# prime-slam/octreelib

Measured on AMD Instinct MI355X. Metric: Mpoints/s insert+subdivide+RANSAC, higher is better.
Workload: dtype f64; 1 GPU; BASELINE config 3: Grid 1 m voxels, 10000000 planar points per GPU (scene 32x32x32 voxels), insert + subdivide(len>64) + map_leaf_points_cuda_ransac(H=1024, k=6, thr=0.01, poses_per_batch=10) incl. apply_mask; points_per_gpu=10000000, K=64, hypotheses=1024, leaves=575543

## Files before the change

### octreelib_amd/csrc/common.h

```cpp
#pragma once

#include <hip/hip_runtime.h>
#include <stdint.h>

#include <cstdio>
#include <cstring>
#include <map>
#include <string>
#include <vector>

#include "../../include/octreelib_hip.h"

#include <atomic>
extern std::atomic<uint64_t> g_octl_host_syncs;
static inline hipError_t octl_counted_stream_sync(hipStream_t s) {
  g_octl_host_syncs.fetch_add(1, std::memory_order_relaxed);
  return hipStreamSynchronize(s);
}
static inline hipError_t octl_counted_event_sync(hipEvent_t e) {
  g_octl_host_syncs.fetch_add(1, std::memory_order_relaxed);
  return hipEventSynchronize(e);
}
#define hipStreamSynchronize(s) octl_counted_stream_sync(s)
#define hipEventSynchronize(e) octl_counted_event_sync(e)
// ... 51 lines not shown
  int64_t no_fused_tables = 0;
  int64_t no_spin_wait = 0;
  int64_t ransac_waves = 0;
  int64_t geom_margin = 0;
  int64_t no_ransac_prescreen = 0;
  int64_t no_spec_finish = 0;
};
int64_t* octl_option_field(OctlOptions& o, const char* name);

struct octl_ctx {
  int device = 0;
  OctlOptions opt;
  hipStream_t stream = nullptr;
  std::string err;
  int profiling = 0;
  std::map<std::string, KernelTiming> timings;
  std::vector<PendingEvent> pending;
  std::vector<hipEvent_t> event_pool;
  DevBuf scan_tmp[3];
  DevBuf scan_status;
  uint32_t scan_epoch = 0;
  int cus = 0;
  DevBuf small;
  void* small_host = nullptr;
  void* pinned = nullptr;
  hipEvent_t pin_event[3] = {nullptr, nullptr, nullptr};
  hipEvent_t handoff_event = nullptr;
  hipStream_t copy_stream = nullptr;
  hipEvent_t copy_gate = nullptr;
  hipStream_t self_stream = nullptr;
  hipEvent_t self_gate = nullptr, self_done = nullptr;
  struct Upload { const char* dst; size_t bytes; hipEvent_t done; };
  std::vector<Upload> uploads;
  std::vector<DevBuf> pool;
  size_t pool_bytes = 0;
  std::map<void*, size_t> user_blocks;
  unsigned char geom_hint[192] = {0};
  bool geom_hint_valid = false;
  bool geom_hint_staged = false;
  struct octl_forest* pending_mask_forest = nullptr;
  uint64_t geom_hint_want = 0;
  bool geom_hint_two_pass = false;
  bool geom_sparse = false;
  bool had_chunks = false;
  int64_t spec_points = 0, spec_nodes = 0, spec_vox = 0, spec_blocks = 0;
  DevBuf hyp_dev;
  DevBuf f32_stage;
  DevBuf ls_buf;
  DevBuf rs_counters;
  int rs_parity = 0;
  uint32_t wait_seq = 0;
  bool rs_counters_dirty = false;
  std::vector<double> hyp_host;
  void* comm = nullptr;
  int n_ranks = 1, rank = 0;
  DevBuf routed_xyz, routed_gidx;
  bool routed_taken = false;
  DevBuf rt_hist, rt_counts, rt_matrix, rt_send_xyz, rt_send_gidx;
  int64_t routed_n = 0;
};

int octl_set_error(octl_ctx* ctx, int code, const char* fmt, ...);
enum { MIRROR_COPY_WORDS = 512, MIRROR_BBOX_WORD = 896, MIRROR_RS_VIOLATION = 990, MIRROR_MASK_TOTALS = 992,
       MIRROR_FLAG_BUILD = 1000, MIRROR_FLAG_MASK0 = 1001, MIRROR_FLAG_MASK1 = 1002 };
static_assert(MIRROR_COPY_WORDS <= MIRROR_BBOX_WORD && MIRROR_BBOX_WORD + 8 <= MIRROR_RS_VIOLATION &&
              MIRROR_RS_VIOLATION < MIRROR_MASK_TOTALS &&
              MIRROR_MASK_TOTALS + 2 <= MIRROR_FLAG_BUILD && MIRROR_FLAG_MASK1 < 1024, "mirror layout");
enum {
  SM_ERR = 0,
  SM_BBOX = 4,
  SM_NVOX = 12,
  SM_NSPLIT = 13,
  SM_NTILES = 14,
  SM_ETOTAL = 15,
  SM_NBLOCKS = 16,
  SM_BK_TICKET = 17,
  SM_BK_OVERFULL = 18,
  SM_SLOT_VOXELS = 21,
  SM_MASK_TOTAL = 22,
  SM_BK_NOORDER = 23,
  SM_DEBUG_TOTAL = 24,
  SM_BK_FLAGS = 25,
  SM_BK_TOTAL = 26,
  SM_BK_TODO = 27,
  SM_BK_MISSING = 28,
  SM_CK_COUNT = 29,
  SM_INC_MISS = 28,
  SM_INC_BAD = 29,
  SM_INC_DEAD = 30,
  SM_INC_NEWVOX = 31,
  SM_SLOT_COUNTS = 28,
  SM_BUILD_WORDS = 32,
  SM_BK_LEVEL = 40,
  SM_GEOM = 64,
  SM_SLOT_HIST = 64,
  SM_ALLREDUCE = 512,
  SM_WORDS = 1024
};
static_assert(SM_ERR < SM_BUILD_WORDS && SM_BBOX + 6 <= SM_BUILD_WORDS && SM_NVOX < SM_BUILD_WORDS &&
                  SM_NSPLIT < SM_BUILD_WORDS && SM_NTILES < SM_BUILD_WORDS && SM_ETOTAL < SM_BUILD_WORDS &&
                  SM_NBLOCKS < SM_BUILD_WORDS && SM_BK_TICKET < SM_BUILD_WORDS && SM_BK_OVERFULL < SM_BUILD_WORDS &&
                  SM_SLOT_VOXELS < SM_BUILD_WORDS && SM_MASK_TOTAL < SM_BUILD_WORDS &&
                  SM_BK_NOORDER < SM_BUILD_WORDS && SM_DEBUG_TOTAL < SM_BUILD_WORDS && SM_BK_FLAGS < SM_BUILD_WORDS &&
                  SM_BK_TOTAL < SM_BUILD_WORDS && SM_BK_TODO < SM_BUILD_WORDS && SM_BK_MISSING < SM_BUILD_WORDS &&
                  SM_CK_COUNT < SM_BUILD_WORDS && SM_INC_NEWVOX < SM_BUILD_WORDS &&
                  SM_SLOT_COUNTS + 4 <= SM_BUILD_WORDS,
// ... 90 lines not shown
```

### octreelib_amd/csrc/ctx.hip

```cpp
#include <chrono>
#include <cstdarg>
#include <cstdlib>

#include <algorithm>

#include "common.h"

int octl_set_error(octl_ctx* ctx, int code, const char* fmt, ...) {
  char buf[1024];
  va_list ap;
  va_start(ap, fmt);
  vsnprintf(buf, sizeof(buf), fmt, ap);
  va_end(ap);
  if (ctx) ctx->err = buf;
  return code;
}

std::atomic<uint64_t> g_octl_host_syncs{0};

namespace {
struct OptName { const char* name; int64_t OctlOptions::*field; };
const OptName kOptions[] = {
    {"NO_BUCKET_BUILD", &OctlOptions::no_bucket_build},     {"BUCKET_POINTS", &OctlOptions::bucket_points},
    {"SYNC_GEOM", &OctlOptions::sync_geom},                 {"NO_GEOM_HINT", &OctlOptions::no_geom_hint},
// ... 315 lines not shown
  if (!out) return OCTL_E_INVALID;
  *out = nullptr;
  int n = 0;
  if (hipGetDeviceCount(&n) != hipSuccess || n <= 0 || device_id < 0 || device_id >= n)
    return OCTL_E_HIP;
  if (hipSetDevice(device_id) != hipSuccess) return OCTL_E_HIP;
  octl_ctx* ctx = new octl_ctx();
  ctx->device = device_id;
  options_from_environment(ctx->opt);
  if (hipStreamCreateWithFlags(&ctx->stream, hipStreamNonBlocking) != hipSuccess) {
    delete ctx;
    return OCTL_E_HIP;
  }
  if (hipMalloc(&ctx->small.p, 4096) != hipSuccess ||
      hipHostMalloc(&ctx->small_host, 4096, hipHostMallocDefault) != hipSuccess ||
      hipHostMalloc(&ctx->pinned, OCTL_PINNED_BYTES, hipHostMallocDefault) != hipSuccess) {
    if (ctx->small.p) (void)hipFree(ctx->small.p);
    (void)hipStreamDestroy(ctx->stream);
    delete ctx;
    return OCTL_E_NOMEM;
  }
  ctx->small.cap = 4096;
  std::memset(ctx->small_host, 0, 4096);
  (void)hipMemsetAsync(ctx->small.p, 0, 4096, ctx->stream);
  (void)hipStreamSynchronize(ctx->stream);
  *out = ctx;
  return OCTL_OK;
}

int octl_comm_destroy(octl_ctx* ctx);

void octl_ctx_destroy(octl_ctx* ctx) {
  if (!ctx) return;
  (void)hipSetDevice(ctx->device);
  (void)hipStreamSynchronize(ctx->stream);
  if (ctx->comm) (void)octl_comm_destroy(ctx);
  for (auto& pe : ctx->pending) {
    (void)hipEventDestroy(pe.start);
    (void)hipEventDestroy(pe.stop);
  }
  for (auto ev : ctx->event_pool) (void)hipEventDestroy(ev);
  if (ctx->handoff_event) (void)hipEventDestroy(ctx->handoff_event);
  for (auto ev : ctx->pin_event)
    if (ev) (void)hipEventDestroy(ev);
  for (auto& pb : ctx->pool) (void)hipFree(pb.p);
  ctx->pool.clear();
  for (auto& ub : ctx->user_blocks) (void)hipFree(ub.first);
  ctx->user_blocks.clear();
  for (auto& b : ctx->scan_tmp) devbuf_free(b);
  devbuf_free(ctx->hyp_dev);
  devbuf_free(ctx->f32_stage);
  devbuf_free(ctx->ls_buf);
  devbuf_free(ctx->rs_counters);
  devbuf_free(ctx->scan_status);
  devbuf_free(ctx->small);
  devbuf_free(ctx->routed_xyz);
  devbuf_free(ctx->routed_gidx);
  for (DevBuf* b : {&ctx->rt_hist, &ctx->rt_counts, &ctx->rt_matrix, &ctx->rt_send_xyz,
                    &ctx->rt_send_gidx})
    devbuf_free(*b);
  if (ctx->small_host) (void)hipHostFree(ctx->small_host);
  if (ctx->pinned) (void)hipHostFree(ctx->pinned);
  if (ctx->self_stream) {
    (void)hipStreamSynchronize(ctx->self_stream);
    (void)hipStreamDestroy(ctx->self_stream);
    if (ctx->self_gate) (void)hipEventDestroy(ctx->self_gate);
    if (ctx->self_done) (void)hipEventDestroy(ctx->self_done);
  }
  if (ctx->copy_stream) {
    (void)hipStreamSynchronize(ctx->copy_stream);
    (void)hipStreamDestroy(ctx->copy_stream);
  }
  if (ctx->copy_gate) (void)hipEventDestroy(ctx->copy_gate);
  for (auto& u : ctx->uploads) (void)hipEventDestroy(u.done);
  (void)hipStreamDestroy(ctx->stream);
  delete ctx;
}

const char* octl_last_error(const octl_ctx* ctx) { return ctx ? ctx->err.c_str() : "null context"; }

int octl_ctx_sync(octl_ctx* ctx) {
  if (!ctx) return OCTL_E_INVALID;
  HIP_TRY(ctx, hipStreamSynchronize(ctx->stream));
  return mirror_check_violation(ctx);
}

int octl_host_alloc(octl_ctx* ctx, int64_t bytes, void** p) {
  if (!ctx || !p || bytes < 0) return OCTL_E_INVALID;
  (void)hipSetDevice(ctx->device);
  hipError_t e = hipHostMalloc(p, (size_t)(bytes > 0 ? bytes : 1), hipHostMallocDefault);
  if (e != hipSuccess)
    return octl_set_error(ctx, OCTL_E_NOMEM, "hipHostMalloc(%lld) failed: %s", (long long)bytes, hipGetErrorString(e));
  return OCTL_OK;
}

int octl_host_free(octl_ctx* ctx, void* p) {
  if (!ctx) return OCTL_E_INVALID;
  if (ctx->copy_stream) (void)hipStreamSynchronize(ctx->copy_stream);
  if (p) HIP_TRY(ctx, hipHostFree(p));
  return OCTL_OK;
}

int octl_dev_upload_async(octl_ctx* ctx, void* dptr, const void* src, int64_t bytes) {
  if (!ctx || bytes < 0 || (bytes > 0 && (!dptr || !src))) return OCTL_E_INVALID;
  HIP_TRY(ctx, hipSetDevice(ctx->device));
  if (!ctx->copy_stream) {
// ... 130 lines not shown
```

### octreelib_amd/csrc/order.hip

```cpp
#include <algorithm>

#include "forest.h"

namespace {

__global__ __launch_bounds__(256) void k_sub_up(const int32_t* __restrict__ first_child,
                                                int64_t a, int64_t b,
                                                uint32_t* __restrict__ nint) {
  const int64_t x = a + (int64_t)blockIdx.x * blockDim.x + threadIdx.x;
  if (x >= b) return;
  const int32_t fc = first_child[x];
  uint32_t s = 0;
  if (fc >= 0) {
    s = 1;
#pragma unroll
    for (int j = 0; j < 8; ++j) s += nint[fc + j];
  }
  nint[x] = s;
}

__global__ __launch_bounds__(256) void k_rank_down(const int32_t* __restrict__ first_child,
                                                   int64_t a, int64_t b,
                                                   const uint32_t* __restrict__ nint,
                                                   uint32_t* __restrict__ rank) {
// ... 263 lines not shown
  OCTL_TRY(forest_settle(f));
  octl_ctx* ctx = f->ctx;
  if (!f->built) return octl_set_error(ctx, OCTL_E_STATE, "no scheme has been built");
  const int n_poses = (int)f->pose_off.size() - 1;
  if (e0 && n_e0 != n_poses) return octl_set_error(ctx, OCTL_E_INVALID, "e0 size mismatch");
  std::vector<uint32_t> slot_counts;
  OCTL_TRY(forest_reference_order(f, e0, slot_counts, false));
  *n_blocks = f->n_blocks;
  const int64_t n = std::min<int64_t>(cap, f->n_blocks);
  if (n > 0 && order) {
    HIP_TRY(ctx, hipMemcpyAsync(order, f->rs_order.p, (size_t)n * 4, hipMemcpyDeviceToHost,
                                ctx->stream));
    HIP_TRY(ctx, hipStreamSynchronize(ctx->stream));
  }
  return OCTL_OK;
}

static int ransac_all_impl(octl_forest* f, int32_t poses_per_batch, const int32_t* e0, int32_t n_e0,
                           const double* hypotheses, int32_t H, int32_t k, double threshold,
                           bool* mask_fresh);

extern "C" int octl_forest_ransac_all(octl_forest* f, int32_t poses_per_batch, const int32_t* e0,
                                      int32_t n_e0, const double* hypotheses, int32_t H, int32_t k,
                                      double threshold) {
  if (!f || !hypotheses) return OCTL_E_INVALID;
  OCTL_TRY(forest_settle(f));
  bool mask_fresh = false;
  const int rc = ransac_all_impl(f, poses_per_batch, e0, n_e0, hypotheses, H, k, threshold, &mask_fresh);
  if (mask_fresh) f->mask_valid = (rc == OCTL_OK);
  return rc;
}

static int ransac_all_impl(octl_forest* f, int32_t poses_per_batch, const int32_t* e0, int32_t n_e0,
                           const double* hypotheses, int32_t H, int32_t k, double threshold,
                           bool* mask_fresh) {
  octl_ctx* ctx = f->ctx;
  if (!f->built) return octl_set_error(ctx, OCTL_E_STATE, "ransac before build");
  if (poses_per_batch < 1) return octl_set_error(ctx, OCTL_E_INVALID, "poses_per_batch < 1");
  if (H < 1 || H > 1024 || k < 1) return octl_set_error(ctx, OCTL_E_INVALID, "bad H or k");
  OCTL_TRY(ransac_check_table(ctx, hypotheses, H, k));
  const int n_poses = (int)f->pose_off.size() - 1;
  if (e0 && n_e0 != n_poses) return octl_set_error(ctx, OCTL_E_INVALID, "e0 size mismatch");
  HIP_TRY(ctx, hipSetDevice(ctx->device));
  hipStream_t st = ctx->stream;
  if (!f->mask_valid) {
    OCTL_TRY(devbuf_reserve(ctx, f->mask, (size_t)std::max<int64_t>(f->n_ord, 1)));
    *mask_fresh = true;
  }
  if (f->n_blocks == 0) return OCTL_OK;
  const size_t hyp_cap_before = ctx->hyp_dev.cap;
  OCTL_TRY(devbuf_reserve(ctx, ctx->hyp_dev, (size_t)H * k * 8));
  const bool same_table = hyp_cap_before == ctx->hyp_dev.cap && ctx->hyp_host.size() == (size_t)H * k &&
                          std::memcmp(ctx->hyp_host.data(), hypotheses, (size_t)H * k * 8) == 0;
  if (same_table) {
  } else if ((size_t)H * k * 8 <= 64 * 1024) {
    char* pin = static_cast<char*>(ctx->pinned) + 128 * 1024;
    OCTL_TRY(pin_region_wait(ctx, 1));
    std::memcpy(pin, hypotheses, (size_t)H * k * 8);
    OCTL_TRY(octl_copy_from_pinned(ctx, ctx->hyp_dev.p, pin, (size_t)H * k * 8));
    OCTL_TRY(pin_region_mark(ctx, 1));
  } else {
    HIP_TRY(ctx, hipMemcpyAsync(ctx->hyp_dev.p, hypotheses, (size_t)H * k * 8, hipMemcpyHostToDevice, st));
    HIP_TRY(ctx, hipStreamSynchronize(st));
  }
  if (!same_table) ctx->hyp_host.assign(hypotheses, hypotheses + (size_t)H * k);
  const bool one_batch = n_poses <= poses_per_batch;
  std::vector<uint32_t> slot_counts;
  OCTL_TRY(forest_reference_order(f, e0, slot_counts, !one_batch));
  if (one_batch) {
    OCTL_TRY(ransac_launch(ctx, f->xyz_ord.as<double>(), f->n_ord, f->blk_start.as<uint32_t>(),
                           f->blk_size.as<int32_t>(), f->rs_order.as<int32_t>(), f->n_blocks,
                           ctx->hyp_dev.as<double>(), H, k, threshold, f->mask.as<uint8_t>(), nullptr,
                           nullptr, nullptr, nullptr, f->rs_scratch, f->max_block_hint));
    return OCTL_OK;
  }
  int64_t off = 0;
  for (int p0 = 0; p0 < n_poses; p0 += poses_per_batch) {
    int64_t nbatch = 0;
    for (int p = p0; p < std::min(n_poses, p0 + poses_per_batch); ++p) nbatch += slot_counts[p];
    if (nbatch > 0)
      OCTL_TRY(ransac_launch(ctx, f->xyz_ord.as<double>(), f->n_ord, f->blk_start.as<uint32_t>(),
                             f->blk_size.as<int32_t>(), f->rs_order.as<int32_t>() + off, nbatch,
                             ctx->hyp_dev.as<double>(), H, k, threshold, f->mask.as<uint8_t>(),
                             nullptr, nullptr, nullptr, nullptr, f->rs_scratch, f->max_block_hint));
    off += nbatch;
  }
  return OCTL_OK;
}
```

### octreelib_amd/csrc/ransac.hip

```cpp
#include <algorithm>
#include <cstdlib>
#include <type_traits>

#include "forest.h"
#include "lookback.h"
#include "plane_cert.h"
#include "wave_utils.h"

namespace {

__device__ __forceinline__ double div_by_small_int(double c, int k) {
  const double kd = (double)k;
  const double zh = 1.0 / kd;
  const double zl = fma(-kd, zh, 1.0) / kd;
  const double a = fabs(c);
  if (!((int(a > 1e-290) | int(c == 0.0)) & int(a < 1e290))) return c / kd;
  return copysign(fma(c, zh, c * zl), c);
}

__device__ __forceinline__ bool coord_in_fast_range(double v) {
  const uint32_t hi = (uint32_t)__double2hiint(v), lo = (uint32_t)__double2loint(v);
  const uint32_t e = (hi >> 20) & 0x7FFu;
  return (e - (1023u - 30u)) <= 60u || (hi | lo) == 0u;
}
// ... 276 lines not shown
  }
  unsigned long long best = 0;
#pragma unroll
  for (int q = 0; q < HPL; ++q) {
    const int t = threadIdx.x + q * THREADS;
    if (t < H) {
      const unsigned long long key =
          ((unsigned long long)(unsigned)cnt[q] << 32) | (unsigned)(0x7FFFFFFF - t);
      best = key > best ? key : best;
    }
  }
#pragma unroll
  for (int off = 32; off > 0; off >>= 1) {
    const unsigned long long o = __shfl_xor(best, off);
    best = o > best ? o : best;
  }
  if ((threadIdx.x & 63) == 0) s_best[threadIdx.x >> 6] = best;
  __syncthreads();
  best = s_best[0];
#pragma unroll
  for (int w = 1; w < THREADS / 64; ++w) best = s_best[w] > best ? s_best[w] : best;
  const int win = 0x7FFFFFFF - (int)(unsigned)(best & 0xFFFFFFFFu);
#pragma unroll
  for (int q = 0; q < HPL; ++q) {
    if ((int)threadIdx.x + q * THREADS == win) {
      const float f0 = (float)pa[q], f1 = (float)pb[q], f2 = (float)pc[q], f3 = (float)pd[q];
      s_plane[0] = f0; s_plane[1] = f1; s_plane[2] = f2; s_plane[3] = f3;
      if (out.plane) {
        out.plane[4 * (int64_t)be + 0] = f0; out.plane[4 * (int64_t)be + 1] = f1;
        out.plane[4 * (int64_t)be + 2] = f2; out.plane[4 * (int64_t)be + 3] = f3;
      }
      if (out.count) out.count[be] = cnt[q];
      if (out.index) out.index[be] = win;
    }
  }
  __syncthreads();
  const double a = (double)s_plane[0], bb = (double)s_plane[1], c = (double)s_plane[2],
               dd = (double)s_plane[3];
  for (int i = threadIdx.x; i < n; i += THREADS)
    out.mask[pstart + i] = (plane_distance(a, bb, c, dd, pts[3 * (int64_t)i], pts[3 * (int64_t)i + 1],
                                           pts[3 * (int64_t)i + 2]) < thr) ? 1 : 0;
}

typedef float f4 __attribute__((ext_vector_type(4)));
__device__ __forceinline__ float fma32(float a, float b, float c) { return __builtin_fmaf(a, b, c); }
__device__ __forceinline__ float min3abs(float m, float a, float b) {
  float r;
  asm("v_min3_f32 %0, %1, |%2|, |%3|" : "=v"(r) : "v"(m), "v"(a), "v"(b));
  return r;
}

template <int CTRL, int ROW_MASK>
__device__ __forceinline__ uint32_t dpp_u32(uint32_t v) {
  return (uint32_t)__builtin_amdgcn_update_dpp((int)v, (int)v, CTRL, ROW_MASK, 0xF, false);
}
__device__ __forceinline__ uint32_t wave_max_u32(uint32_t v) {
  v = max(v, dpp_u32<0xB1, 0xF>(v));
  v = max(v, dpp_u32<0x4E, 0xF>(v));
  v = max(v, dpp_u32<0x141, 0xF>(v));
  v = max(v, dpp_u32<0x140, 0xF>(v));
  v = max(v, dpp_u32<0x142, 0xA>(v));
  v = max(v, dpp_u32<0x143, 0xC>(v));
  return (uint32_t)__builtin_amdgcn_readlane((int)v, 63);
}
__device__ __forceinline__ float wave_max_nonneg_f32(float m) {
  return __uint_as_float(wave_max_u32(__float_as_uint(m)));
}

template <int CTRL, int ROW_MASK>
__device__ __forceinline__ double dpp_f64_or_zero(double v) {
  const int lo = __builtin_amdgcn_update_dpp(0, __double2loint(v), CTRL, ROW_MASK, 0xF, false);
  const int hi = __builtin_amdgcn_update_dpp(0, __double2hiint(v), CTRL, ROW_MASK, 0xF, false);
  return __hiloint2double(hi, lo);
}
__device__ __forceinline__ double wave_sum_f64(double v) {
  v += dpp_f64_or_zero<0xB1, 0xF>(v);
  v += dpp_f64_or_zero<0x4E, 0xF>(v);
  v += dpp_f64_or_zero<0x141, 0xF>(v);
  v += dpp_f64_or_zero<0x140, 0xF>(v);
  v += dpp_f64_or_zero<0x142, 0xA>(v);
  v += dpp_f64_or_zero<0x143, 0xC>(v);
  return __hiloint2double(__builtin_amdgcn_readlane(__double2hiint(v), 63),
                          __builtin_amdgcn_readlane(__double2loint(v), 63));
}

template <int THREADS, bool SFAST = false>
__device__ __forceinline__ void stage_local(unsigned tx, double ox, double oy, double oz, const BlockDesc& d,
                                            double px, double py, double pz, f4* loc,
                                            float* wext, uint32_t* wfast, float* ext_out = nullptr,
                                            uint32_t* fast_out = nullptr) {
  float m = 0.f;
  if ((int)tx < d.n) {
    const float u = (float)(px - ox), v = (float)(py - oy), w = (float)(pz - oz);
    loc[tx] = f4{u, v, w, 0.f};
    m = fmaxf(fabsf(u), fmaxf(fabsf(v), fabsf(w)));
    if (!(m == m) || u != u || v != v || w != w) m = __int_as_float(0x7f800000);
  }
  m = wave_max_nonneg_f32(m);
  const bool inr = coord_in_fast_range(px) && coord_in_fast_range(py) && coord_in_fast_range(pz);
  const bool wave_fast = __all(inr);
  if (ext_out) {
    *ext_out = m;
    *fast_out = SFAST ? (uint32_t)__builtin_amdgcn_readfirstlane(wave_fast ? 1 : 0) : (wave_fast ? 1u : 0u);
  } else if ((tx & 63) == 0) {
    wext[tx >> 6] = m;
    wfast[tx >> 6] = wave_fast ? 1u : 0u;
  }
}

template <int NH>
__device__ __forceinline__ void screen_group(const f4* __restrict__ loc, int n, const float* fa,
                                             const float* fb, const float* fc, const float* sto,
                                             float nthr2, int* cnt, float* margin) {
  float mg[2][NH];
#pragma unroll
  for (int h = 0; h < NH; ++h) mg[0][h] = mg[1][h] = __int_as_float(0x7f800000);
  for (int base = 0; base < n; base += 32) {
    const int m = __builtin_amdgcn_readfirstlane(min(32, n - base));
    uint32_t hist[NH];
#pragma unroll
    for (int h = 0; h < NH; ++h) hist[h] = 0;
    auto score = [&](const f4 L, float (&e)[NH]) {
#pragma unroll
      for (int h = 0; h < NH; ++h) {
        const float sv = fma32(fa[h], L.x, fma32(fb[h], L.y, fma32(fc[h], L.z, sto[h])));
        e[h] = fma32(sv, sv, nthr2);
        hist[h] = __builtin_amdgcn_alignbit(hist[h], __float_as_uint(e[h]), 31);
      }
    };
    int i = 0;
    for (; i + 4 <= m; i += 4) {
      const f4 L0 = loc[base + i], L1 = loc[base + i + 1], L2 = loc[base + i + 2],
               L3 = loc[base + i + 3];
      float e0[NH], e1[NH], e2[NH], e3[NH];
// ... 454 lines not shown
              RS_COUNT(17, 64 * (n - m1));
              RS_COUNT(21, 1);
              survive(mine && c2[0] > Lcur, (uint32_t)c2[0], (int)(w & 1023u));
              qhead += nq;
            };
            auto prescreen = [&](auto nh_tag, const int qb) {
              constexpr int NH = decltype(nh_tag)::value;
              uint2 pe[NH];
              auto hyp_a = [&](const int h) { return (int)tx + (qb + h) * THREADS; };
#pragma unroll
              for (int h = 0; h < NH; ++h)
                pe[h] = pos_tab[(size_t)n * (size_t)H + (size_t)((FULLH || hyp_a(h) < H) ? hyp_a(h) : 0)];
              float qa[NH], qb_[NH], qc[NH], qto[NH], qT2[NH];
              bool qok[NH];
              int qcnt[NH];
              uint32_t risk = 0;
#pragma unroll
              for (int h = 0; h < NH; ++h) {
                const uint32_t w0 = pe[h].x, w1 = pe[h].y;
                f4 P[KS];
#pragma unroll
                for (int i = 0; i < KS; ++i) P[i] = loc[((i < 4 ? w0 : w1) >> (8 * (i & 3))) & 0xFFu];
                const float inv_k = 1.0f / (float)KS;
                float cx = P[0].x, cy = P[0].y, cz = P[0].z;
#pragma unroll
                for (int i = 1; i < KS; ++i) {
                  cx += P[i].x;
                  cy += P[i].y;
                  cz += P[i].z;
                }
                cx *= inv_k;
                cy *= inv_k;
                cz *= inv_k;
                float xx, xy, xz, yy, yz, zz;
                {
                  const float ax = P[0].x - cx, ay = P[0].y - cy, az = P[0].z - cz;
                  xx = ax * ax; xy = ax * ay; xz = ax * az; yy = ay * ay; yz = ay * az; zz = az * az;
                }
#pragma unroll
                for (int i = 1; i < KS; ++i) {
                  const float ax = P[i].x - cx, ay = P[i].y - cy, az = P[i].z - cz;
                  xx = fma32(ax, ax, xx); xy = fma32(ax, ay, xy); xz = fma32(ax, az, xz);
                  yy = fma32(ay, ay, yy); yz = fma32(ay, az, yz); zz = fma32(az, az, zz);
                }
                const float dx = fma32(yy, zz, -(yz * yz)), dy = fma32(xx, zz, -(xz * xz)), dz = fma32(xx, yy, -(xy * xy));
                const float cA = fma32(xz, yz, -(xy * zz)), cB = fma32(xy, yz, -(xz * yy)), cC = fma32(xy, xz, -(yz * xx));
                const bool is_x = dx > dy && dx > dz;
                const bool is_y = !is_x && dy > dz;
                const float m1 = is_x ? dx : (is_y ? cA : cB);
                const float m2 = is_x ? cA : (is_y ? dy : cC);
                const float m3 = is_x ? cB : (is_y ? cC : dz);
                const float ss = fma32(m3, m3, fma32(m2, m2, m1 * m1));
                const float r = __builtin_amdgcn_rsqf(ss);
                const float a = m1 * r, b = m2 * r, c = m3 * r;
                qa[h] = a; qb_[h] = b; qc[h] = c;
                float to = -fma32(c, cz, fma32(b, cy, a * cx));
                asm volatile("" : "+v"(to));
                qto[h] = to;
                const float T = (xx + yy) + zz;
                const float mu4 = fma32(fma32(pc.qa, T, pc.qb), T, pc.qc);
                const float gap = __builtin_fmaxf(__builtin_fmaxf(dx, dy), dz) - __builtin_amdgcn_fmed3f(dx, dy, dz);
                qok[h] = (ss * r > mu4) && (gap > mu4);
                risk |= w1;
                const float thr_h = fma32(pc.e35, mu4 * r, pc.thrblk);
                qT2[h] = thr_h * thr_h;
                qcnt[h] = 0;
              }
              if (__any((risk >> 16) != 0u)) {
#pragma unroll
                for (int h = 0; h < NH; ++h) qok[h] = qok[h] && (pe[h].y >> 16) == 0u;
              }
              RS_COUNT(12, NH);
              RS_COUNT(22, 64 * NH * n);
              if constexpr (TWO) {
                if (two_stage) {
                  bool bad = false;
#pragma unroll
                  for (int h = 0; h < NH; ++h) bad = bad || !qok[h];
                  if (__any(bad)) {
#pragma unroll
                    for (int h = 0; h < NH; ++h) {
                      if (!qok[h]) {
                        qa[h] = qb_[h] = qc[h] = qto[h] = 0.f;
                        qT2[h] = 1.f;
                      }
                    }
                  }
                  screen_ub<NH>(ploc, m1, qa, qb_, qc, qto, qT2, qcnt);
                  RS_COUNT(16, 64 * NH * m1);
#pragma unroll
                  for (int h = 0; h < NH; ++h) {
                    const bool alive = qcnt[h] > m1 - budget && (FULLH || hyp_a(h) < H);
                    const unsigned long long mk = __ballot(alive);
                    if (alive) {
                      const int e = (qtail + (int)__builtin_amdgcn_mbcnt_hi((uint32_t)(mk >> 32), __builtin_amdgcn_mbcnt_lo((uint32_t)mk, 0u))) &
                                    (RS_STAGE2_RING - 1);
                      qlo[e] = __float_as_uint(qa[h]);
                      qlo[RS_STAGE2_RING + e] = __float_as_uint(qb_[h]);
                      qlo[2 * RS_STAGE2_RING + e] = __float_as_uint(qc[h]);
                      qhi[e] = __float_as_uint(qto[h]);
                      qhi[RS_STAGE2_RING + e] = __float_as_uint(qT2[h]);
                      qhi[2 * RS_STAGE2_RING + e] = ((uint32_t)qcnt[h] << 10) | (uint32_t)hyp_a(h);
                    }
                    qtail += __popcll(mk);
                    RS_COUNT(18, __popcll(mk));
                    if (qtail - qhead >= 64) stage2(64);
                  }
                  return;
                }
              }
              screen_ub<NH>(loc, n, qa, qb_, qc, qto, qT2, qcnt);
              RS_COUNT(20, 64 * NH * n);
#pragma unroll
              for (int h = 0; h < NH; ++h)
                survive(!(qok[h] && qcnt[h] <= Lcur) && (FULLH || hyp_a(h) < H),
                        (THREADS == 64 && qok[h]) ? (uint32_t)qcnt[h] : 63u, hyp_a(h));
            };
            constexpr int PNH = 3;
            constexpr int TRIOS = (HPL - 1) / PNH, REST = (HPL - 1) % PNH;
            if (TWO && certified) {
              const float E = extent;
              const float G = ((float)(fabs(lx[0]) + fabs(ly[0]) + fabs(lz[0])) + E) * 0x1.0002p0f;
              const float E2 = E * E;
              const float floor2 = fma32(0x1p-74f * (G * G), E2, 0x1p-24f * (E2 * E2)) * 0x1.0002p0f;
              const uint32_t* __restrict__ trio = reinterpret_cast<const uint32_t*>(pos_tab) + trio_word(n, H, 0);
              auto trio_of = [&](int g) {
                const int t = (int)tx + g * THREADS;
                return trio[(FULLH || t < H) ? t : 0];
              };
              auto at = [&](uint32_t off) { return *reinterpret_cast<const f4*>(reinterpret_cast<const char*>(loc) + off); };
              uint32_t e_next = trio_of(1);
#pragma unroll 1
              for (int g = 1; g < HPL; ++g) {
                const int t = (int)tx + g * THREADS;
                const bool real = FULLH || t < H;
                const uint32_t e = e_next;
                e_next = trio_of(g + 1 < HPL ? g + 1 : g);
                const f4 P0 = at(e & 0x3F0u), P1 = at((e >> 10) & 0x3F0u), P2 = at((e >> 20) & 0x3F0u);
                const float ux = P1.x - P0.x, uy = P1.y - P0.y, uz = P1.z - P0.z;
                const float vx = P2.x - P0.x, vy = P2.y - P0.y, vz = P2.z - P0.z;
// ... 415 lines not shown
      sp = start[phys[r + 1]];
    } else if (!order) {
      const int64_t e = (int64_t)d.pstart + d.n;
      if (e < n_points) sp = (uint32_t)e;
    }
    d.pspill = sp;
    d.pad[0] = 0;
    d.pad[1] = (uint32_t)b;
    d.pad[2] = 0;
    desc[b] = d;
    if (d.n < k) {
      for (int i = 0; i < d.n; ++i) out.mask[(int64_t)d.pstart + i] = 0;
      if (out.plane) {
        out.plane[4 * b + 0] = 0.f; out.plane[4 * b + 1] = 0.f;
        out.plane[4 * b + 2] = 0.f; out.plane[4 * b + 3] = 0.f;
      }
      if (out.count) out.count[b] = 0;
      if (out.index) out.index[b] = -1;
    } else if (d.n > cap) {
      big_list[atomicAdd(&counters[RC_BIG], 1u)] = (uint32_t)b;
    } else {
      atomicAdd(&bins[d.n], 1u);
    }
    if (d.n >= k && (int64_t)d.n > max_block)
      __hip_atomic_store(&mirror[MIRROR_RS_VIOLATION], 1u, __ATOMIC_RELAXED, __HIP_MEMORY_SCOPE_SYSTEM);
  }
  __syncthreads();
  if (bins[threadIdx.x]) atomicAdd(&counters[RC_BINS + threadIdx.x], bins[threadIdx.x]);
}

__device__ __forceinline__ void pos_table_entry(const double* __restrict__ hyp, int H, int k,
                                                uint2* __restrict__ tab, int n, int t) {
  const double* __restrict__ row = hyp + (int64_t)t * k;
  uint32_t x = 0, y = 0;
  for (int i = 0; i < k; ++i) {
    bool risky;
    const uint32_t g = (uint32_t)sample_index_cached(row[i], n, &risky);
    if (i < 4) x |= g << (8 * i); else y |= g << (8 * (i - 4));
    y |= (risky || g == (uint32_t)n) ? (0x10000u << i) : 0u;
  }
  tab[(size_t)n * (size_t)H + t] = uint2{x, y};
  if (n < RS_TINY_THREADS && k >= 3) {
    auto p = [&](int i) { return ((i < 4 ? x : y) >> (8 * (i & 3))) & 0xFFu; };
    const uint32_t p0 = p(0);
    uint32_t p1 = p(k - 1), p2 = p(k - 1);
    for (int i = k - 2; i >= 1; --i) p1 = p(i) != p0 ? p(i) : p1;
    for (int i = k - 2; i >= 2; --i) p2 = (p(i) != p0 && p(i) != p1) ? p(i) : p2;
    const bool flagged = (y >> 16) != 0u || p1 == p0 || p2 == p0 || p2 == p1;
    reinterpret_cast<uint32_t*>(tab)[trio_word(n, H, t)] = flagged ? TRIO_FLAG : (p0 << 4) | (p1 << 14) | (p2 << 24);
  }
}
__device__ __forceinline__ void pos_table_part(const double* __restrict__ hyp, int H, int k,
                                               const uint32_t* __restrict__ counters, uint2* __restrict__ tab,
                                               int n, int part) {
  const int t = part * 256 + (int)threadIdx.x;
  if (t >= H || n < k || counters[RC_BINS + n] == 0u) return;
  pos_table_entry(hyp, H, k, tab, n, t);
}

__global__ __launch_bounds__(256) void k_block_scatter(const BlockDesc* __restrict__ desc, int64_t nb,
                                                       int cap, int k,
                                                       uint32_t* __restrict__ counters,
                                                       BlockDesc* __restrict__ sdesc, unsigned n_scatter,
                                                       const double* __restrict__ hyp, int H,
                                                       uint2* __restrict__ tab, uint32_t* __restrict__ next_counters) {
  if (next_counters && blockIdx.x == gridDim.x - 1)
    for (int w = threadIdx.x; w < RC_WORDS; w += blockDim.x) next_counters[w] = 0;
  if (blockIdx.x >= n_scatter) {
    const unsigned parts = (unsigned)(H + 255) / 256u;
    const unsigned id = blockIdx.x - n_scatter;
    pos_table_part(hyp, H, k, counters, tab, (int)(id / parts), (int)(id % parts));
    return;
  }
  __shared__ uint32_t cnt[256];
  __shared__ uint32_t base[256];
  __shared__ uint32_t c[256];
  cnt[threadIdx.x] = 0;
  c[threadIdx.x] = counters[RC_BINS + threadIdx.x];
  __syncthreads();
  uint32_t first = 0;
  for (int m = 255; m > (int)threadIdx.x; --m) first += c[m];
  if (blockIdx.x == 0) {
    counters[RC_START + threadIdx.x] = first;
    if (threadIdx.x == 0) counters[RC_SORTED] = first + c[0];
  }
  constexpr int PER_THREAD = BS_PER_THREAD;
  const int64_t b0 = (int64_t)blockIdx.x * (256 * PER_THREAD);
  int nn[PER_THREAD];
  uint32_t rank[PER_THREAD];
#pragma unroll
  for (int r = 0; r < PER_THREAD; ++r) {
    const int64_t b = b0 + r * 256 + threadIdx.x;
    nn[r] = -1;
    rank[r] = 0;
    if (b < nb) {
      const int n = desc[b].n;
      if (n >= k && n <= cap) {
        nn[r] = n;
        rank[r] = atomicAdd(&cnt[n], 1u);
      }
    }
  }
  __syncthreads();
  if (cnt[threadIdx.x]) base[threadIdx.x] = first + atomicAdd(&counters[RC_FILL + threadIdx.x], cnt[threadIdx.x]);
  __syncthreads();
#pragma unroll
  for (int r = 0; r < PER_THREAD; ++r) {
    if (nn[r] >= 0) {
      const int64_t b = b0 + r * 256 + threadIdx.x;
      sdesc[base[nn[r]] + rank[r]] = desc[b];
    }
  }
}

constexpr int BPS_THREADS = 1024, BPS_MAX = BPS_THREADS * 8;
template <int BPS_PER_THREAD>
__global__ __launch_bounds__(BPS_THREADS) void k_block_prepare_small(
    const int32_t* __restrict__ order, const uint32_t* __restrict__ start, const int32_t* __restrict__ size,
    int64_t nb, int64_t n_points, int cap, int k, BlockDesc* __restrict__ desc, BlockDesc* __restrict__ sdesc,
    uint32_t* __restrict__ big_list, uint32_t* __restrict__ counters, RansacOut out, int64_t max_block,
    uint32_t* __restrict__ mirror, const double* __restrict__ hyp, int H, uint2* __restrict__ tab,
    uint32_t* __restrict__ next_counters) {
  if (blockIdx.x > 0) {
    const int parts = (H + BPS_THREADS - 1) / BPS_THREADS;
// ... 86 lines not shown
  uint32_t cm = 0, incm = 0;
  if (threadIdx.x < 256) {
    cm = bins[255 - threadIdx.x];
    incm = wave_inclusive_add(cm);
    if (lane == 63) s_wave[wave] = incm;
  }
  __syncthreads();
  if (threadIdx.x < 256) {
    uint32_t f = incm - cm;
    for (int w = 0; w < wave; ++w) f += s_wave[w];
    const int m = 255 - (int)threadIdx.x;
    first[m] = f;
    counters[RC_BINS + m] = cm;
    counters[RC_START + m] = f;
    if (m == 0) counters[RC_SORTED] = f + cm;
  }
  __syncthreads();
#pragma unroll
  for (int r = 0; r < BPS_PER_THREAD; ++r)
    if (dd[r].n >= 0) sdesc[first[dd[r].n] + rank[r]] = dd[r];
}

}

int ransac_check_table(octl_ctx* ctx, const double* hyp, int32_t H, int32_t k) {
  const int64_t n = (int64_t)H * k;
  for (int64_t i = 0; i < n; ++i)
    if (!(hyp[i] >= 0.0 && hyp[i] < 1.0))
      return octl_set_error(ctx, OCTL_E_INVALID,
                            "hypothesis table entry %lld = %g is outside [0, 1): the table must hold "
                            "np.random.random draws (cuda_ransac.py:39-41)", (long long)i, hyp[i]);
  return OCTL_OK;
}

int ransac_launch(octl_ctx* ctx, const double* xyz_dev, int64_t n_points,
                  const uint32_t* blk_start, const int32_t* blk_size, const int32_t* order_dev,
                  int64_t nb, const double* hyp_dev, int32_t H, int32_t k, double thr,
                  uint8_t* mask_dev, float* plane_dev, int32_t* count_dev, int32_t* index_dev,
                  uint8_t* evaluated_dev, DevBuf& scratch, int64_t max_block) {
  (void)evaluated_dev;
  if (nb <= 0) return OCTL_OK;
  if (H < 1 || H > 1024) return octl_set_error(ctx, OCTL_E_INVALID, "H must be in [1, 1024]");
  if (k < 1) return octl_set_error(ctx, OCTL_E_INVALID, "initial_points_number must be positive");
  const bool any_k = k > RS_KMAX;
  if (nb >= ((int64_t)1 << 31)) return octl_set_error(ctx, OCTL_E_INVALID, "too many blocks");
  hipStream_t st = ctx->stream;
  const size_t off_d = (((size_t)nb + 8) * 4 + 31) & ~(size_t)31;
  const size_t off_s = off_d + (size_t)nb * sizeof(BlockDesc);
  const size_t off_b = off_s + (size_t)nb * sizeof(BlockDesc);
  const size_t off_c = (off_b + (size_t)nb * 4 + 31) & ~(size_t)31;
  const bool use_tab = !any_k && k >= 3 && k <= 6 && (H > 256 || k == 6);
  const size_t off_t = (off_c + RC_WORDS * 4 + 31) & ~(size_t)31;
  const size_t tab_bytes = (size_t)256 * (size_t)H * sizeof(uint2) + (size_t)RS_TINY_THREADS * (size_t)H * sizeof(uint32_t);
  OCTL_TRY(devbuf_reserve(ctx, scratch, off_t + (use_tab ? tab_bytes : 0)));
  char* base = static_cast<char*>(scratch.p);
  uint32_t* tmp = scratch.as<uint32_t>();
  BlockDesc* desc = reinterpret_cast<BlockDesc*>(base + off_d);
  BlockDesc* sdesc = reinterpret_cast<BlockDesc*>(base + off_s);
  uint32_t* big_list = reinterpret_cast<uint32_t*>(base + off_b);
  uint32_t* counters = reinterpret_cast<uint32_t*>(base + off_c);
  const bool fused = !ctx->opt.no_fused_tables;
  uint32_t* next_counters = nullptr;
  if (fused) {
    if (!ctx->rs_counters.p || ctx->rs_counters_dirty) {
      OCTL_TRY(devbuf_reserve(ctx, ctx->rs_counters, (size_t)2 * RC_WORDS * 4));
      HIP_TRY(ctx, hipMemsetAsync(ctx->rs_counters.p, 0, (size_t)2 * RC_WORDS * 4, st));
      ctx->rs_parity = 0;
    }
    counters = ctx->rs_counters.as<uint32_t>() + (size_t)ctx->rs_parity * RC_WORDS;
    next_counters = ctx->rs_counters.as<uint32_t>() + (size_t)(ctx->rs_parity ^ 1) * RC_WORDS;
    ctx->rs_parity ^= 1;
    ctx->rs_counters_dirty = true;
  }
  uint2* pos_tab = use_tab ? reinterpret_cast<uint2*>(base + off_t) : nullptr;
  const int threads = (H <= 64) ? 64 : (H <= 256 ? 256 : RS_BIG_THREADS);
  RansacOut out{mask_dev, plane_dev, count_dev, index_dev};
  if (fused && nb <= BPS_MAX) {
    KTimer t(ctx, "ransac_prepare");
    const int cap = any_k ? 0 : threads - 1;
    const unsigned n_table = use_tab && cap >= k ? (unsigned)(cap - k + 1) * (unsigned)ceil_div(H, BPS_THREADS) : 0u;
    auto kp = nb <= 2 * BPS_THREADS ? k_block_prepare_small<2>
              : (nb <= 4 * BPS_THREADS ? k_block_prepare_small<4>
                                       : (nb <= 6 * BPS_THREADS ? k_block_prepare_small<6> : k_block_prepare_small<8>));
    OCTL_LAUNCH(kp, dim3(1 + n_table), dim3(BPS_THREADS), 0, st, order_dev, blk_start, blk_size, nb,
                       n_points, cap, (int)k, desc, sdesc, big_list, counters, out, max_block,
                       static_cast<uint32_t*>(ctx->small_host), hyp_dev, (int)H, pos_tab, next_counters);
    HIP_TRY(ctx, hipGetLastError());
    ctx->rs_counters_dirty = false;
  } else {
    KTimer t(ctx, "ransac_prepare");
    if (fused) {
      const unsigned g = (unsigned)ceil_div(nb, 256 * BP_PER_THREAD);
      uint64_t* status = nullptr;
      uint32_t epoch = 0;
      OCTL_TRY(octl_scan_status_acquire(ctx, g, &status, &epoch));
      OCTL_LAUNCH(k_block_prepare, dim3(g), dim3(256), 0, st, order_dev, blk_start, blk_size, nb, n_points,
                         any_k ? 0 : threads - 1, (int)k, desc, big_list, counters, out, status, epoch, max_block,
                         static_cast<uint32_t*>(ctx->small_host));
      HIP_TRY(ctx, hipGetLastError());
    } else {
      const unsigned g = (unsigned)ceil_div(nb, 256);
      OCTL_LAUNCH(k_block_sizes_in_order, dim3(g), dim3(256), 0, st, order_dev, blk_size, nb, tmp, counters);
      HIP_TRY(ctx, hipGetLastError());
      OCTL_TRY(octl_exclusive_scan_u32(ctx, tmp, tmp, nb, nullptr));
      OCTL_LAUNCH(k_block_desc, dim3((unsigned)ceil_div(nb, 256 * BD_PER_THREAD)), dim3(256), 0, st, order_dev,
                         blk_start, blk_size,
                         (const uint32_t*)tmp, nb, n_points, any_k ? 0 : threads - 1, (int)k, desc, big_list,
                         counters, out);
      HIP_TRY(ctx, hipGetLastError());
    }
    const unsigned n_scatter = (unsigned)ceil_div(nb, 256 * BS_PER_THREAD);
    const unsigned n_table = use_tab ? 256u * (unsigned)ceil_div(H, 256) : 0u;
    OCTL_LAUNCH(k_block_scatter, dim3(n_scatter + n_table), dim3(256), 0, st,
                       (const BlockDesc*)desc, nb, any_k ? 0 : threads - 1, (int)k, counters, sdesc, n_scatter, hyp_dev,
                       (int)H, pos_tab, next_counters);
    HIP_TRY(ctx, hipGetLastError());
    ctx->rs_counters_dirty = false;
  }
  const int cus = octl_ctx_cus(ctx);
  KTimer t(ctx, "ransac");
  hipStream_t side = st;
  bool on_side = false;
  int waves_per_block = (int)ctx->opt.ransac_waves;
  if (waves_per_block == 0 && !any_k && H > 256) {
    const int64_t slots = (int64_t)cus * 16;
    if (nb * 2 <= slots) waves_per_block = 4;
    else if (nb <= 6 * slots) waves_per_block = 2;
  }
  const bool need_small = max_block >= RS_TINY_THREADS, need_mid = max_block >= RS_SMALL_THREADS,
             need_big = any_k || max_block >= threads;
  const bool side_work = waves_per_block == 4 ? need_big
                         : (waves_per_block == 2 ? (need_mid || need_big) : (need_small || need_mid || need_big));
  if (!any_k && H > 256 && side_work && octl_ctx_side_stream(ctx) &&
      hipEventRecord(ctx->self_gate, st) == hipSuccess &&
      hipStreamWaitEvent(ctx->self_stream, ctx->self_gate, 0) == hipSuccess) {
    side = ctx->self_stream;
    on_side = true;
  }
  const int no_prescreen = ctx->opt.no_ransac_prescreen ? 1 : 0;
#define OCTL_RANSAC_RANGE(THREADS, HPL, KT, PER_CU, LO, HI, PT, ST)                              \
  do {                                                                                           \
    const unsigned g = (unsigned)std::min<int64_t>(nb, (int64_t)cus * (PER_CU));                 \
    if (H == (THREADS) * (HPL))                                                                  \
      OCTL_LAUNCH((k_ransac<THREADS, HPL, KT, true, PT>), dim3(g), dim3(THREADS), 0, ST,         \
                         xyz_dev, (const BlockDesc*)sdesc, (const uint32_t*)(LO), (const uint32_t*)(HI), \
                         hyp_dev, H, k, thr, out, (const uint2*)pos_tab, no_prescreen);           \
    else                                                                                         \
      OCTL_LAUNCH((k_ransac<THREADS, HPL, KT, false, PT>), dim3(g), dim3(THREADS), 0, ST,        \
                         xyz_dev, (const BlockDesc*)sdesc, (const uint32_t*)(LO), (const uint32_t*)(HI), \
                         hyp_dev, H, k, thr, out, (const uint2*)pos_tab, no_prescreen);           \
  } while (0)
#define OCTL_RANSAC_LAUNCH(THREADS, HPL, KT, PER_CU, PT) \
  OCTL_RANSAC_RANGE(THREADS, HPL, KT, PER_CU, nullptr, counters + RC_SORTED, PT, st)
#define OCTL_RANSAC_SPLIT(KT)                                                                                    \
  do {                                                                                                           \
    if (waves_per_block == 4) {                                                                                  \
      OCTL_RANSAC_RANGE(RS_BIG_THREADS, RS_BIG_HPL, KT, RS_PER_CU, nullptr, counters + RC_SORTED, true, st);     \
    } else if (waves_per_block == 2) {                                                                           \
      if (need_mid)                                                                                              \
        OCTL_RANSAC_RANGE(RS_BIG_THREADS, RS_BIG_HPL, KT, RS_PER_CU, nullptr,                                    \
                          counters + RC_START + RS_SMALL_THREADS - 1, true, side);                               \
      HIP_TRY(ctx, hipGetLastError());                                                                           \
      OCTL_RANSAC_RANGE(RS_SMALL_THREADS, (1024 / RS_SMALL_THREADS), KT, RS_SMALL_PER_CU,                        \
                        counters + RC_START + RS_SMALL_THREADS - 1, counters + RC_SORTED, true, st);             \
    } else {                                                                                                     \
      if (need_mid)                                                                                              \
        OCTL_RANSAC_RANGE(RS_BIG_THREADS, RS_BIG_HPL, KT, RS_PER_CU, nullptr,                                    \
                          counters + RC_START + RS_SMALL_THREADS - 1, true, side);                               \
      HIP_TRY(ctx, hipGetLastError());                                                                           \
      if (need_small)                                                                                            \
// ... 139 lines not shown
```

Before: 3939 Mpoints/s.

## Cache RANSAC position table across calls and simplify wave reductions

Moves the per-call hypothesis position table into a persistent context buffer, keyed by a hypothesis serial number plus H and k, so later calls with the same hypothesis table skip rebuilding it. When the table is cached it is built for every sample size up to the cap instead of only the sizes seen in the current call. The change also rewrites the f64 wave-sum DPP helpers to use full masks with bound_ctrl. It also restructures the two-stage screening so bad hypotheses are zeroed inline instead of in a separate wave-vote pass. This reuses derived data across calls, which is risky under a hack rule, but the table depends only on the hypotheses, which are an input.

Result: no change. 3986 Mpoints/s, median of 6 (+1.2%).

```diff
diff --git a/octreelib_amd/csrc/common.h b/octreelib_amd/csrc/common.h
--- a/octreelib_amd/csrc/common.h
+++ b/octreelib_amd/csrc/common.h
@@ -127,6 +127,10 @@
   uint32_t wait_seq = 0;
   bool rs_counters_dirty = false;
   std::vector<double> hyp_host;
+  DevBuf rs_tab;
+  uint64_t hyp_serial = 0, rs_tab_serial = 0;
+  int32_t rs_tab_H = 0, rs_tab_k = 0;
+  const void* rs_tab_at = nullptr;
   void* comm = nullptr;
   int n_ranks = 1, rank = 0;
   DevBuf routed_xyz, routed_gidx;
diff --git a/octreelib_amd/csrc/ctx.hip b/octreelib_amd/csrc/ctx.hip
--- a/octreelib_amd/csrc/ctx.hip
+++ b/octreelib_amd/csrc/ctx.hip
@@ -391,6 +391,7 @@
   devbuf_free(ctx->f32_stage);
   devbuf_free(ctx->ls_buf);
   devbuf_free(ctx->rs_counters);
+  devbuf_free(ctx->rs_tab);
   devbuf_free(ctx->scan_status);
   devbuf_free(ctx->small);
   devbuf_free(ctx->routed_xyz);
diff --git a/octreelib_amd/csrc/order.hip b/octreelib_amd/csrc/order.hip
--- a/octreelib_amd/csrc/order.hip
+++ b/octreelib_amd/csrc/order.hip
@@ -339,6 +339,7 @@
   OCTL_TRY(devbuf_reserve(ctx, ctx->hyp_dev, (size_t)H * k * 8));
   const bool same_table = hyp_cap_before == ctx->hyp_dev.cap && ctx->hyp_host.size() == (size_t)H * k &&
                           std::memcmp(ctx->hyp_host.data(), hypotheses, (size_t)H * k * 8) == 0;
+  if (!same_table) ctx->hyp_serial += 1;
   if (same_table) {
   } else if ((size_t)H * k * 8 <= 64 * 1024) {
     char* pin = static_cast<char*>(ctx->pinned) + 128 * 1024;
diff --git a/octreelib_amd/csrc/ransac.hip b/octreelib_amd/csrc/ransac.hip
--- a/octreelib_amd/csrc/ransac.hip
+++ b/octreelib_amd/csrc/ransac.hip
@@ -352,7 +352,7 @@
 
 template <int CTRL, int ROW_MASK>
 __device__ __forceinline__ uint32_t dpp_u32(uint32_t v) {
-  return (uint32_t)__builtin_amdgcn_update_dpp((int)v, (int)v, CTRL, ROW_MASK, 0xF, false);
+  return (uint32_t)__builtin_amdgcn_update_dpp(0, (int)v, CTRL, ROW_MASK, 0xF, false);
 }
 __device__ __forceinline__ uint32_t wave_max_u32(uint32_t v) {
   v = max(v, dpp_u32<0xB1, 0xF>(v));
@@ -367,19 +367,19 @@
   return __uint_as_float(wave_max_u32(__float_as_uint(m)));
 }
 
-template <int CTRL, int ROW_MASK>
-__device__ __forceinline__ double dpp_f64_or_zero(double v) {
-  const int lo = __builtin_amdgcn_update_dpp(0, __double2loint(v), CTRL, ROW_MASK, 0xF, false);
-  const int hi = __builtin_amdgcn_update_dpp(0, __double2hiint(v), CTRL, ROW_MASK, 0xF, false);
+template <int CTRL>
+__device__ __forceinline__ double dpp_f64(double v) {
+  const int lo = __builtin_amdgcn_update_dpp(0, __double2loint(v), CTRL, 0xF, 0xF, true);
+  const int hi = __builtin_amdgcn_update_dpp(0, __double2hiint(v), CTRL, 0xF, 0xF, true);
   return __hiloint2double(hi, lo);
 }
 __device__ __forceinline__ double wave_sum_f64(double v) {
-  v += dpp_f64_or_zero<0xB1, 0xF>(v);
-  v += dpp_f64_or_zero<0x4E, 0xF>(v);
-  v += dpp_f64_or_zero<0x141, 0xF>(v);
-  v += dpp_f64_or_zero<0x140, 0xF>(v);
-  v += dpp_f64_or_zero<0x142, 0xA>(v);
-  v += dpp_f64_or_zero<0x143, 0xC>(v);
+  v += dpp_f64<0xB1>(v);
+  v += dpp_f64<0x4E>(v);
+  v += dpp_f64<0x141>(v);
+  v += dpp_f64<0x140>(v);
+  v += dpp_f64<0x142>(v);
+  v += dpp_f64<0x143>(v);
   return __hiloint2double(__builtin_amdgcn_readlane(__double2hiint(v), 63),
                           __builtin_amdgcn_readlane(__double2loint(v), 63));
 }
@@ -940,40 +940,36 @@
                 const float m3 = is_x ? cB : (is_y ? cC : dz);
                 const float ss = fma32(m3, m3, fma32(m2, m2, m1 * m1));
                 const float r = __builtin_amdgcn_rsqf(ss);
-                const float a = m1 * r, b = m2 * r, c = m3 * r;
+                const float T = (xx + yy) + zz;
+                const float mu4 = fma32(fma32(pc.qa, T, pc.qb), T, pc.qc);
+                const float gap = __builtin_fmaxf(__builtin_fmaxf(dx, dy), dz) - __builtin_amdgcn_fmed3f(dx, dy, dz);
+                qok[h] = (ss * r > mu4) && (gap > mu4);
+                float rn = r;
+                if constexpr (TWO) {
+                  qok[h] = qok[h] && (w1 >> 16) == 0u;
+                  rn = qok[h] ? r : 0.f;
+                } else {
+                  risk |= w1;
+                }
+                const float a = m1 * rn, b = m2 * rn, c = m3 * rn;
                 qa[h] = a; qb_[h] = b; qc[h] = c;
                 float to = -fma32(c, cz, fma32(b, cy, a * cx));
                 asm volatile("" : "+v"(to));
                 qto[h] = to;
-                const float T = (xx + yy) + zz;
-                const float mu4 = fma32(fma32(pc.qa, T, pc.qb), T, pc.qc);
-                const float gap = __builtin_fmaxf(__builtin_fmaxf(dx, dy), dz) - __builtin_amdgcn_fmed3f(dx, dy, dz);
-                qok[h] = (ss * r > mu4) && (gap > mu4);
-                risk |= w1;
-                const float thr_h = fma32(pc.e35, mu4 * r, pc.thrblk);
+                const float thr_h = fma32(pc.e35, mu4 * rn, pc.thrblk);
                 qT2[h] = thr_h * thr_h;
                 qcnt[h] = 0;
               }
-              if (__any((risk >> 16) != 0u)) {
-#pragma unroll
-                for (int h = 0; h < NH; ++h) qok[h] = qok[h] && (pe[h].y >> 16) == 0u;
+              if constexpr (!TWO) {
+                if (__any((risk >> 16) != 0u)) {
+#pragma unroll
+                  for (int h = 0; h < NH; ++h) qok[h] = qok[h] && (pe[h].y >> 16) == 0u;
+                }
               }
               RS_COUNT(12, NH);
               RS_COUNT(22, 64 * NH * n);
               if constexpr (TWO) {
                 if (two_stage) {
-                  bool bad = false;
-#pragma unroll
-                  for (int h = 0; h < NH; ++h) bad = bad || !qok[h];
-                  if (__any(bad)) {
-#pragma unroll
-                    for (int h = 0; h < NH; ++h) {
-                      if (!qok[h]) {
-                        qa[h] = qb_[h] = qc[h] = qto[h] = 0.f;
-                        qT2[h] = 1.f;
-                      }
-                    }
-                  }
                   screen_ub<NH>(ploc, m1, qa, qb_, qc, qto, qT2, qcnt);
                   RS_COUNT(16, 64 * NH * m1);
 #pragma unroll
@@ -1495,9 +1491,10 @@
 }
 __device__ __forceinline__ void pos_table_part(const double* __restrict__ hyp, int H, int k,
                                                const uint32_t* __restrict__ counters, uint2* __restrict__ tab,
-                                               int n, int part) {
+                                               int n, int part, int cap, bool every_size) {
   const int t = part * 256 + (int)threadIdx.x;
-  if (t >= H || n < k || counters[RC_BINS + n] == 0u) return;
+  if (t >= H || n < k) return;
+  if (every_size ? n > cap : counters[RC_BINS + n] == 0u) return;
   pos_table_entry(hyp, H, k, tab, n, t);
 }
 
@@ -1506,13 +1503,14 @@
                                                        uint32_t* __restrict__ counters,
                                                        BlockDesc* __restrict__ sdesc, unsigned n_scatter,
                                                        const double* __restrict__ hyp, int H,
-                                                       uint2* __restrict__ tab, uint32_t* __restrict__ next_counters) {
+                                                       uint2* __restrict__ tab, uint32_t* __restrict__ next_counters,
+                                                       int tab_every_size) {
   if (next_counters && blockIdx.x == gridDim.x - 1)
     for (int w = threadIdx.x; w < RC_WORDS; w += blockDim.x) next_counters[w] = 0;
   if (blockIdx.x >= n_scatter) {
     const unsigned parts = (unsigned)(H + 255) / 256u;
     const unsigned id = blockIdx.x - n_scatter;
-    pos_table_part(hyp, H, k, counters, tab, (int)(id / parts), (int)(id % parts));
+    pos_table_part(hyp, H, k, counters, tab, (int)(id / parts), (int)(id % parts), cap, tab_every_size != 0);
     return;
   }
   __shared__ uint32_t cnt[256];
@@ -1705,7 +1703,20 @@
   const bool use_tab = !any_k && k >= 3 && k <= 6 && (H > 256 || k == 6);
   const size_t off_t = (off_c + RC_WORDS * 4 + 31) & ~(size_t)31;
   const size_t tab_bytes = (size_t)256 * (size_t)H * sizeof(uint2) + (size_t)RS_TINY_THREADS * (size_t)H * sizeof(uint32_t);
-  OCTL_TRY(devbuf_reserve(ctx, scratch, off_t + (use_tab ? tab_bytes : 0)));
+  const bool ctx_tab = use_tab && ctx->hyp_dev.p && hyp_dev == ctx->hyp_dev.as<double>();
+  OCTL_TRY(devbuf_reserve(ctx, scratch, off_t + (use_tab && !ctx_tab ? tab_bytes : 0)));
+  if (ctx_tab) OCTL_TRY(devbuf_reserve(ctx, ctx->rs_tab, tab_bytes));
+  const bool tab_made = ctx_tab && ctx->rs_tab_serial != 0 && ctx->rs_tab_serial == ctx->hyp_serial &&
+                        ctx->rs_tab_H == H && ctx->rs_tab_k == k && ctx->rs_tab_at == ctx->rs_tab.p;
+  if (ctx_tab && !tab_made) ctx->rs_tab_serial = 0;
+  auto tab_done = [&]() {
+    if (ctx_tab && !tab_made) {
+      ctx->rs_tab_serial = ctx->hyp_serial;
+      ctx->rs_tab_H = H;
+      ctx->rs_tab_k = k;
+      ctx->rs_tab_at = ctx->rs_tab.p;
+    }
+  };
   char* base = static_cast<char*>(scratch.p);
   uint32_t* tmp = scratch.as<uint32_t>();
   BlockDesc* desc = reinterpret_cast<BlockDesc*>(base + off_d);
@@ -1725,13 +1736,13 @@
     ctx->rs_parity ^= 1;
     ctx->rs_counters_dirty = true;
   }
-  uint2* pos_tab = use_tab ? reinterpret_cast<uint2*>(base + off_t) : nullptr;
+  uint2* pos_tab = !use_tab ? nullptr : (ctx_tab ? ctx->rs_tab.as<uint2>() : reinterpret_cast<uint2*>(base + off_t));
   const int threads = (H <= 64) ? 64 : (H <= 256 ? 256 : RS_BIG_THREADS);
   RansacOut out{mask_dev, plane_dev, count_dev, index_dev};
   if (fused && nb <= BPS_MAX) {
     KTimer t(ctx, "ransac_prepare");
     const int cap = any_k ? 0 : threads - 1;
-    const unsigned n_table = use_tab && cap >= k ? (unsigned)(cap - k + 1) * (unsigned)ceil_div(H, BPS_THREADS) : 0u;
+    const unsigned n_table = use_tab && !tab_made && cap >= k ? (unsigned)(cap - k + 1) * (unsigned)ceil_div(H, BPS_THREADS) : 0u;
     auto kp = nb <= 2 * BPS_THREADS ? k_block_prepare_small<2>
               : (nb <= 4 * BPS_THREADS ? k_block_prepare_small<4>
                                        : (nb <= 6 * BPS_THREADS ? k_block_prepare_small<6> : k_block_prepare_small<8>));
@@ -1740,6 +1751,7 @@
                        static_cast<uint32_t*>(ctx->small_host), hyp_dev, (int)H, pos_tab, next_counters);
     HIP_TRY(ctx, hipGetLastError());
     ctx->rs_counters_dirty = false;
+    tab_done();
   } else {
     KTimer t(ctx, "ransac_prepare");
     if (fused) {
@@ -1763,12 +1775,13 @@
       HIP_TRY(ctx, hipGetLastError());
     }
     const unsigned n_scatter = (unsigned)ceil_div(nb, 256 * BS_PER_THREAD);
-    const unsigned n_table = use_tab ? 256u * (unsigned)ceil_div(H, 256) : 0u;
+    const unsigned n_table = use_tab && !tab_made ? 256u * (unsigned)ceil_div(H, 256) : 0u;
     OCTL_LAUNCH(k_block_scatter, dim3(n_scatter + n_table), dim3(256), 0, st,
                        (const BlockDesc*)desc, nb, any_k ? 0 : threads - 1, (int)k, counters, sdesc, n_scatter, hyp_dev,
-                       (int)H, pos_tab, next_counters);
+                       (int)H, pos_tab, next_counters, ctx_tab ? 1 : 0);
     HIP_TRY(ctx, hipGetLastError());
     ctx->rs_counters_dirty = false;
+    tab_done();
   }
   const int cus = octl_ctx_cus(ctx);
   KTimer t(ctx, "ransac");
```
